# maoqingyu1996/Boosting-Neural-Video-Representation-via-Online-Structural-Reparameteration

Hardware: AMD Instinct MI355X
Metric: training frames/sec, Bunny 720p ERB (higher is better)
Workload: dtype f16; 1 GPU; configs[1]: Bunny-shaped 132x3x720x1280 synthetic video, branch_type=ERB, fc_hw_dim 9_16_26, strides 5 2 2 2 2, stem 512_1, lower_width 96, Fusion6, Adam(0.5,0.999), b=1; one independent video per GPU; precision=fp16, hip_graph=False, launch_mode=stream, finite=True

## Files before the change

boosting-neural-video-representation-via-online-structural-reparameteration_amd/_lib.py:

```python
import ctypes
import os
from ctypes import POINTER, c_char_p, c_double, c_float, c_int, c_int32, c_int64, c_size_t, c_void_p

HERE = os.path.dirname(os.path.abspath(__file__))
ORN_MAX_LAYERS = 8
LOSS_TYPES = {'L2': 0, 'L1': 1, 'Fusion6': 2}


class OrnError(RuntimeError):
    pass


def lib_path() -> str:
    return os.environ.get('ORN_LIB_PATH') or os.path.join(HERE, 'liborn.so')


class LayerDesc(ctypes.Structure):
    _fields_ = [('C', c_int32), ('O', c_int32), ('s', c_int32), ('H', c_int32), ('W', c_int32),
                ('w3x3', c_int64), ('b3x3', c_int64), ('w3x1', c_int64), ('b3x1', c_int64),
                ('w1x3', c_int64), ('b1x3', c_int64), ('w1', c_int64), ('w2', c_int64), ('w3', c_int64)]


class EngineDesc(ctypes.Structure):
    _fields_ = [('n_layers', c_int32), ('erb', c_int32), ('embed_len', c_int32), ('stem_dim', c_int32),
                ('fc_h', c_int32), ('fc_w', c_int32), ('fc_dim', c_int32), ('sigmoid', c_int32),
                ('loss_type', c_int32), ('precision', c_int32),
                ('beta1', c_double), ('beta2', c_double), ('eps', c_double),
                ('stem_w0', c_int64), ('stem_b0', c_int64), ('stem_w1', c_int64), ('stem_b1', c_int64),
                ('head_w', c_int64), ('head_b', c_int64), ('n_params', c_int64),
                ('layer', LayerDesc * ORN_MAX_LAYERS)]


P = c_void_p
_SIGS = {
    'orn_version': (c_int, []),
    'orn_last_error': (c_int, [c_char_p, c_size_t]),
    'orn_pe_fwd': (c_int, [P, c_int, P, c_int, P, P]),
    'orn_stem_fwd': (c_int, [P, P, P, P, P, c_int, c_int, c_int, c_int, P, P, P, P, P]),
    'orn_stem_bwd': (c_int, [P, P, P, P, P, P, c_int, c_int, c_int, c_int, P, P, P, P, P, P]),
    'orn_erb_merge_fwd': (c_int, [P] * 9 + [c_int, c_int, P, P, P, P]),
    'orn_erb_merge_bwd_ws_bytes': (c_size_t, [c_int, c_int]),
    'orn_erb_merge_bwd': (c_int, [P] * 6 + [c_int, c_int] + [P] * 9 + [P, c_size_t, P]),
    'orn_conv3x3_ps_silu_fwd': (c_int, [P, P, P, c_int, c_int, c_int, c_int, c_int, c_int, P, P, P]),
    'orn_conv3x3_ps_silu_bwd_ws_bytes': (c_size_t, [c_int] * 5),
    'orn_conv3x3_ps_silu_bwd': (c_int, [P, P, P, P] + [c_int] * 6 + [P, P, P, P, c_size_t, P]),
    'orn_conv3x3_ps_silu_bf16_ws_bytes': (c_size_t, [c_int] * 5),
    'orn_conv3x3_ps_silu_fwd_bf16': (c_int, [P, P, P] + [c_int] * 5 + [P, P, P, c_size_t, P]),
    'orn_conv3x3_ps_silu_bwd_bf16': (c_int, [P, P, P, P] + [c_int] * 5 + [P, P, P, P, c_size_t, P]),
    'orn_conv_nhwc_bf16_fwd': (c_int, [P, P, P] + [c_int] * 5 + [P, P, P]),
    'orn_conv_nhwc_f16_fwd': (c_int, [P, P, P] + [c_int] * 5 + [P, P, P]),
    'orn_dgrad_nhwc_bf16': (c_int, [P, P] + [c_int] * 4 + [P, P, c_int, P]),
    'orn_wgrad_nhwc_bf16_ws_bytes': (c_size_t, [c_int] * 3),
    'orn_wgrad_nhwc_bf16': (c_int, [P, P] + [c_int] * 5 + [P, P, P, P]),
    'orn_dgrad_nhwc_f16': (c_int, [P, P] + [c_int] * 4 + [P, P, c_int, P]),
    'orn_wgrad_nhwc_f16': (c_int, [P, P] + [c_int] * 5 + [P, P, P, P]),
    'orn_conv3x3_ps_silu_fwd_f16': (c_int, [P, P, P] + [c_int] * 5 + [P, P, P, c_size_t, P]),
    'orn_conv3x3_ps_silu_bwd_f16': (c_int, [P, P, P, P] + [c_int] * 5 + [P, P, P, P, c_size_t, P]),
    'orn_head_fwd': (c_int, [P, P, P, c_int, c_int, c_int, c_int, c_int, P, P]),
    'orn_head_bwd_ws_bytes': (c_size_t, [c_int] * 4),
    'orn_head_bwd': (c_int, [P, P, P, P, c_int, c_int, c_int, c_int, c_int, P, P, P, P, c_size_t, P]),
    'orn_loss_ws_bytes': (c_size_t, [c_int] * 4),
    'orn_loss_fwd_bwd': (c_int, [P, P, c_int, c_int, c_int, c_int, c_int, c_float, P, P, P, c_size_t, P]),
    'orn_loss_target_stats_bytes': (c_size_t, [c_int] * 4),
    'orn_loss_target_stats': (c_int, [P, c_int, c_int, c_int, c_int, P, P]),
    'orn_msssim_ws_bytes': (c_size_t, [c_int] * 4),
    'orn_msssim': (c_int, [P, P, c_int, c_int, c_int, c_int, P, P, c_size_t, P]),
    'orn_adam_step': (c_int, [P, P, P, P, c_size_t, c_double, c_double, c_double, c_double, c_int, P]),
    'orn_engine_ws_bytes': (c_size_t, [POINTER(EngineDesc)]),
    'orn_engine_create': (c_int, [POINTER(EngineDesc), P, P, P, P, P, c_size_t, POINTER(c_void_p)]),
    'orn_engine_destroy': (None, [P]),
    'orn_engine_decode': (c_int, [P, P, P, P]),
    'orn_engine_train_step': (c_int, [P, P, P, P, P, P, c_int32, P]),
    'orn_engine_train_steps_graph': (c_int, [P, P, P, P, P, P, c_int32, c_int32, P]),
    'orn_engine_train_steps': (c_int, [P, P, P, P, P, P, c_int32, c_int32, P]),
    'orn_engine_profile_step': (c_int, [P, P, P, P, P, P, c_int32, P, P]),
    'orn_engine_set_grad_mask': (c_int, [P, P]),
    'orn_engine_set_target_stats': (c_int, [P, P]),
    'orn_engine_fused_kernel': (c_int, [P, c_int, POINTER(c_void_p), POINTER(c_void_p)]),
    'orn_engine_scale_state': (c_int, [P, P]),
    'orn_engine_set_grad_scale': (c_int, [P, c_float, c_float]),
}
EXPORTS = tuple(_SIGS.keys())
_DEBUG_SIGS = {'orn_debug_set': (None, [c_int]), 'orn_debug_set_stamps': (None, [c_void_p]),
               'orn_debug_conv_fwd_bf16': (c_int, [P, P, P] + [c_int] * 5 + [P, P, c_int, P]),
               'orn_debug_conv_fwd_f16': (c_int, [P, P, P] + [c_int] * 5 + [P, P, c_int, P]),
               'orn_debug_conv_dgrad_bf16': (c_int, [P, P] + [c_int] * 4 + [P, P, c_int, P, c_int, P]),
               'orn_debug_conv_dgrad_f16': (c_int, [P, P] + [c_int] * 4 + [P, P, c_int, P, c_int, P]),
               'orn_debug_merge_h16_bwd': (c_int, [c_int, P, P, P, P, P])}

_lib = None


def lib():
    global _lib
    if _lib is None:
        path = lib_path()
        if not os.path.exists(path):
            raise OrnError(f'{path} is missing: build it with `python -c "import __graft_entry__ as g; g.build()"` '
                           '(hipcc --offload-arch=gfx950).  There is no CPU fallback.')
        L = ctypes.CDLL(path)
        for name, (res, args) in _SIGS.items():
            fn = getattr(L, name)
            fn.restype = res
            fn.argtypes = args
        for name, (res, args) in _DEBUG_SIGS.items():
            fn = getattr(L, name, None)
            if fn is not None:
                fn.restype = res
                fn.argtypes = args
        _lib = L
    return _lib


def last_error() -> str:
    buf = ctypes.create_string_buffer(512)
    lib().orn_last_error(buf, 512)
    return buf.value.decode('utf-8', 'replace')


def check(rc: int, what: str = ''):
    if rc != 0:
        raise OrnError(f'{what or "liborn"} failed (rc={rc}): {last_error()}')


def ptr(t):
    if t is None:
        return None
    if not t.is_cuda:
        raise OrnError('liborn ops need tensors on the GPU (there is no CPU path)')
    if not t.is_contiguous():
        raise OrnError('liborn ops need contiguous tensors')
    return c_void_p(t.data_ptr())


def stream():
    import torch
    return c_void_p(torch.cuda.current_stream().cuda_stream)
```

boosting-neural-video-representation-via-online-structural-reparameteration_amd/csrc/orn_loss.hip:

```cpp
#include "orn_internal.h"

#define SS_TH 16
#define SS_TW 64
#define SS_PH (SS_TH + 10)
#define SS_PW (SS_TW + 10)
#define SS_PWP 76

__constant__ float c_gauss[11];

struct LossP {
    const float *pred, *target;
    const int *frame_idx;
    size_t frame_stride;
    int planes, H, W, Hv, Wv;
    float *part_ssim;
    float *part_l1;
    float *dpred;
    int loss_type;
    int vec4;
    float *tstats;
    size_t tstats_stride;
    float g_l1, g_l2, g_ssim;
    int tiles_w, tiles_h;
};

#define F6_TH 16
#define F6_TW 64
#define F6_PH (F6_TH + 20)
#define F6_PWP 88
#define F6_DH (F6_TH + 10)
#define F6_DWP 76
#define F6_LDS_FLOATS (2 * F6_PH * F6_PWP + 5 * F6_PH * F6_DWP + 16)

enum { TC_NONE = 0, TC_READ = 1, TC_FILL = 2 };
template <bool GRAD, int TC>
__global__ void __launch_bounds__(256) k_fusion6(LossP q)
{
    extern __shared__ __attribute__((aligned(16))) float f6s[];
    float *Xp = f6s, *Xt = f6s + F6_PH * F6_PWP;
    float *Hm = f6s + 2 * F6_PH * F6_PWP;
    float *Dm = f6s;
    float *Hh = Hm;
    float *sred = f6s + 2 * F6_PH * F6_PWP + 5 * F6_PH * F6_DWP;
    const int t = threadIdx.x;
    const int plane = blockIdx.y;
    const int tw = blockIdx.x % q.tiles_w, th = blockIdx.x / q.tiles_w;
    const int y0 = th * F6_TH, x0 = tw * F6_TW;
    const size_t HW = (size_t)q.H * q.W;
    const size_t fr = TC == TC_FILL ? (size_t)blockIdx.z : (q.frame_idx ? (size_t)(*q.frame_idx) : 0);
    const float *tp = q.target + fr * q.frame_stride + (size_t)plane * HW;
    const float *pp = TC == TC_FILL ? tp : q.pred + (size_t)plane * HW;
    float *ts_mu = nullptr, *ts_tt = nullptr;
    if (TC != TC_NONE) {
        ts_mu = q.tstats + fr * q.tstats_stride + (size_t)plane * q.Hv * q.Wv;
        ts_tt = ts_mu + (size_t)q.planes * q.Hv * q.Wv;
    }
    constexpr int RPT = 9;
    const int vrg = t / F6_DWP, vj = t - vrg * F6_DWP, vr4 = vrg == 2 ? 17 : vrg * RPT;
    float c_mu[RPT], c_tt[RPT];
    if (TC == TC_READ && t < 3 * F6_DWP) {
#pragma unroll
        for (int o = 0; o < RPT; ++o) {
            const int vy = min(max(y0 - 10 + vr4 + o, 0), q.Hv - 1), vx = min(max(x0 - 10 + vj, 0), q.Wv - 1);
            c_mu[o] = ts_mu[(size_t)vy * q.Wv + vx];
            c_tt[o] = ts_tt[(size_t)vy * q.Wv + vx];
        }
    }
    if (q.vec4) {
        constexpr int NU = 22, NIT = (F6_PH * NU + 255) / 256;
        float4 ra[NIT], rb[NIT];
#pragma unroll
        for (int it = 0; it < NIT; ++it) {
            const int idx = t + it * 256;
            const int r = idx / NU, u = idx - r * NU;
            const int gy = y0 - 10 + r, gx = x0 - 12 + 4 * u;
            ra[it] = make_float4(0.f, 0.f, 0.f, 0.f); rb[it] = ra[it];
            if (idx < F6_PH * NU && gy >= 0 && gy < q.H && gx >= 0 && gx < q.W) {
                ra[it] = *reinterpret_cast<const float4 *>(pp + (size_t)gy * q.W + gx);
                rb[it] = *reinterpret_cast<const float4 *>(tp + (size_t)gy * q.W + gx);
            }
        }
#pragma unroll
        for (int it = 0; it < NIT; ++it) {
            const int idx = t + it * 256;
            const int r = idx / NU, u = idx - r * NU;
            if (idx < F6_PH * NU) {
                const int c = 4 * u - 2;
                if (u > 0) {
                    *reinterpret_cast<float2 *>(Xp + r * F6_PWP + c) = make_float2(ra[it].x, ra[it].y);
                    *reinterpret_cast<float2 *>(Xt + r * F6_PWP + c) = make_float2(rb[it].x, rb[it].y);
                }
                *reinterpret_cast<float2 *>(Xp + r * F6_PWP + c + 2) = make_float2(ra[it].z, ra[it].w);
                *reinterpret_cast<float2 *>(Xt + r * F6_PWP + c + 2) = make_float2(rb[it].z, rb[it].w);
            }
        }
    } else {
        constexpr int NL = (F6_PH * F6_PWP + 255) / 256;
#pragma unroll 1
        for (int it = 0; it < NL; ++it) {
            const int idx = t + it * 256;
            const int r = idx / F6_PWP, c = idx - r * F6_PWP;
            const int gy = y0 - 10 + r, gx = x0 - 10 + c;
            float a = 0.f, b = 0.f;
            if (idx < F6_PH * F6_PWP && gy >= 0 && gy < q.H && gx >= 0 && gx < q.W) { a = pp[(size_t)gy * q.W + gx]; b = tp[(size_t)gy * q.W + gx]; }
            if (idx < F6_PH * F6_PWP) { Xp[idx] = a; Xt[idx] = b; }
        }
    }
    __syncthreads();
    for (int idx = t; idx < F6_PH * (F6_DWP / 4); idx += 256) {
        const int r = idx / (F6_DWP / 4), c4 = (idx - r * (F6_DWP / 4)) * 4;
        float a[16], b[16];
#pragma unroll
        for (int k = 0; k < 4; ++k) {
            const float4 va = *reinterpret_cast<const float4 *>(Xp + r * F6_PWP + c4 + 4 * k);
            const float4 vb = *reinterpret_cast<const float4 *>(Xt + r * F6_PWP + c4 + 4 * k);
            a[4 * k] = va.x; a[4 * k + 1] = va.y; a[4 * k + 2] = va.z; a[4 * k + 3] = va.w;
            b[4 * k] = vb.x; b[4 * k + 1] = vb.y; b[4 * k + 2] = vb.z; b[4 * k + 3] = vb.w;
        }
        float sp[4] = {0, 0, 0, 0}, st[4] = {0, 0, 0, 0}, spp[4] = {0, 0, 0, 0}, stt[4] = {0, 0, 0, 0}, spt[4] = {0, 0, 0, 0};
        constexpr bool P_MAPS = TC != TC_FILL, T_MAPS = TC != TC_READ;
#pragma unroll
        for (int k = 0; k < 14; ++k) {
            const float aa = a[k] * a[k], bb = b[k] * b[k], ab = a[k] * b[k];
#pragma unroll
            for (int o = 0; o < 4; ++o) {
                const int tap = k - o;
                if (tap >= 0 && tap < 11) {
                    const float g = c_gauss[tap];
                    if (P_MAPS) { sp[o] = fmaf(g, a[k], sp[o]); spp[o] = fmaf(g, aa, spp[o]); spt[o] = fmaf(g, ab, spt[o]); }
                    if (T_MAPS) { st[o] = fmaf(g, b[k], st[o]); stt[o] = fmaf(g, bb, stt[o]); }
                }
            }
        }
        float *h = Hm + r * F6_DWP + c4;
        if (P_MAPS) {
            *reinterpret_cast<float4 *>(h) = make_float4(sp[0], sp[1], sp[2], sp[3]);
            *reinterpret_cast<float4 *>(h + 2 * F6_PH * F6_DWP) = make_float4(spp[0], spp[1], spp[2], spp[3]);
            *reinterpret_cast<float4 *>(h + 4 * F6_PH * F6_DWP) = make_float4(spt[0], spt[1], spt[2], spt[3]);
        }
        if (T_MAPS) {
            *reinterpret_cast<float4 *>(h + F6_PH * F6_DWP) = make_float4(st[0], st[1], st[2], st[3]);
            *reinterpret_cast<float4 *>(h + 3 * F6_PH * F6_DWP) = make_float4(stt[0], stt[1], stt[2], stt[3]);
        }
    }
    __syncthreads();
    const float C1 = 0.01f * 0.01f, C2 = 0.03f * 0.03f;
    float ssum = 0.f;
    if (t < 3 * F6_DWP) {
        const int rg = vrg, j = vj, r4 = vr4;
        float v[5][RPT];
#pragma unroll
        for (int m = 0; m < 5; ++m) {
            if ((TC == TC_READ && (m == 1 || m == 3)) || (TC == TC_FILL && !(m == 1 || m == 3))) continue;
            float col[RPT + 10];
#pragma unroll
            for (int k = 0; k < RPT + 10; ++k) col[k] = Hm[(m * F6_PH + r4 + k) * F6_DWP + j];
#pragma unroll
            for (int o = 0; o < RPT; ++o) {
                float acc = 0.f;
#pragma unroll
                for (int k = 0; k < 11; ++k) acc = fmaf(c_gauss[k], col[o + k], acc);
                v[m][o] = acc;
            }
        }
#pragma unroll
        for (int o = 0; o < RPT; ++o) {
            const int i = r4 + o;
            const int vy = y0 - 10 + i, vx = x0 - 10 + j;
            float dm = 0.f, dq = 0.f, dr = 0.f;
            if (TC == TC_FILL) {
                if (vy >= 0 && vy < q.Hv && vx >= 0 && vx < q.Wv && i >= 10 && j >= 10 && j < F6_TW + 10 && (rg < 2 || o > 0)) {
                    ts_mu[(size_t)vy * q.Wv + vx] = v[1][o];
                    ts_tt[(size_t)vy * q.Wv + vx] = v[3][o];
                }
                continue;
            }
            if (vy >= 0 && vy < q.Hv && vx >= 0 && vx < q.Wv && j < F6_TW + 10) {
                const float m = v[0][o], qq = v[2][o], rr = v[4][o];
                const float mu = TC == TC_READ ? c_mu[o] : v[1][o];
                const float tt = TC == TC_READ ? c_tt[o] : v[3][o];
                const float sp = qq - m * m, st = tt - mu * mu, spt = rr - m * mu;
                const float A1 = 2.f * m * mu + C1, A2 = 2.f * spt + C2;
                const float B1 = m * m + mu * mu + C1, B2 = sp + st + C2;
                float i1 = __builtin_amdgcn_rcpf(B1), i2 = __builtin_amdgcn_rcpf(B2);
                i1 = i1 * (2.0f - B1 * i1);
                i2 = i2 * (2.0f - B2 * i2);
                const float inv = i1 * i2;
                const float S = A1 * A2 * inv;
                if (i >= 10 && j >= 10 && (rg < 2 || o > 0)) ssum += S;
                dm = 2.f * mu * (A2 - A1) * inv - 2.f * m * S * i1 + 2.f * m * S * i2;
                dq = -S * i2;
                dr = 2.f * A1 * inv;
            }
            float *d = Dm + i * F6_DWP + j;
            d[0] = dm; d[F6_DH * F6_DWP] = dq; d[2 * F6_DH * F6_DWP] = dr;
        }
    }
    if (TC == TC_FILL) return;
    const int fc = t & (F6_TW - 1), fr4 = (t >> 6) * 4;
    float fp[4], ft[4];
#pragma unroll
    for (int o = 0; o < 4; ++o) {
        const size_t oo = (size_t)min(y0 + fr4 + o, q.H - 1) * q.W + min(x0 + fc, q.W - 1);
        fp[o] = pp[oo]; ft[o] = tp[oo];
    }
    __syncthreads();
    float sabs = 0.f, ssq = 0.f;
    if (GRAD) {
        for (int idx = t; idx < F6_DH * (F6_TW / 4); idx += 256) {
            const int r = idx / (F6_TW / 4), c4 = (idx - r * (F6_TW / 4)) * 4;
#pragma unroll
            for (int m = 0; m < 3; ++m) {
                float w[16];
#pragma unroll
                for (int k = 0; k < 4; ++k) {
                    const float4 vv = *reinterpret_cast<const float4 *>(Dm + (m * F6_DH + r) * F6_DWP + c4 + 4 * k);
                    w[4 * k] = vv.x; w[4 * k + 1] = vv.y; w[4 * k + 2] = vv.z; w[4 * k + 3] = vv.w;
                }
                float hv[4];
#pragma unroll
                for (int o = 0; o < 4; ++o) {
                    float acc = 0.f;
#pragma unroll
                    for (int k = 0; k < 11; ++k) acc = fmaf(c_gauss[k], w[o + 10 - k], acc);
                    hv[o] = acc;
                }
                *reinterpret_cast<float4 *>(Hh + (m * F6_DH + r) * F6_TW + c4) = make_float4(hv[0], hv[1], hv[2], hv[3]);
            }
        }
        __syncthreads();
    }
    {
        const int c = fc, r4 = fr4;
        float am[4] = {0, 0, 0, 0}, aq[4] = {0, 0, 0, 0}, ar[4] = {0, 0, 0, 0};
        if (GRAD) {
#pragma unroll
            for (int m = 0; m < 3; ++m) {
                float col[14];
#pragma unroll
                for (int k = 0; k < 14; ++k) col[k] = Hh[(m * F6_DH + r4 + k) * F6_TW + c];
#pragma unroll
                for (int o = 0; o < 4; ++o) {
                    float acc = 0.f;
#pragma unroll
                    for (int k = 0; k < 11; ++k) acc = fmaf(c_gauss[k], col[o + 10 - k], acc);
                    if (m == 0) am[o] = acc; else if (m == 1) aq[o] = acc; else ar[o] = acc;
                }
            }
        }
        const int gx = x0 + c;
#pragma unroll
        for (int o = 0; o < 4; ++o) {
            const int gy = y0 + r4 + o;
            if (gy >= q.H || gx >= q.W) continue;
            const size_t oo = (size_t)gy * q.W + gx;
            const float p = fp[o], tg = ft[o], d = p - tg;
            sabs += fabsf(d);
            ssq = fmaf(d, d, ssq);
            if (GRAD) {
                float g = q.g_l1 * ((d > 0.f) ? 1.f : ((d < 0.f) ? -1.f : 0.f));
                g -= q.g_ssim * (am[o] + 2.f * p * aq[o] + tg * ar[o]);
                q.dpred[(size_t)plane * HW + oo] = g;
            }
        }
    }
    const float ts = orn_block_sum(ssum, sred);
    const float ta = orn_block_sum(sabs, sred);
    const float tq = orn_block_sum(ssq, sred);
    if (t == 0) {
        const size_t bi = (size_t)plane * gridDim.x + blockIdx.x;
        q.part_ssim[bi] = ts;
        q.part_l1[2 * bi] = ta;
        q.part_l1[2 * bi + 1] = tq;
    }
}

template <int LT, bool GRAD>
__global__ void __launch_bounds__(256) k_loss_grad(LossP q)
{
    __shared__ float sred[16];
    const int t = threadIdx.x;
    const int plane = blockIdx.y;
    const int tw = blockIdx.x % q.tiles_w, th = blockIdx.x / q.tiles_w;
    const int y0 = th * SS_TH, x0 = tw * SS_TW;
    const size_t HW = (size_t)q.H * q.W;
    const float *pp = q.pred + (size_t)plane * HW;
    const float *tp = q.target + (q.frame_idx ? (size_t)(*q.frame_idx) * q.frame_stride : 0) + (size_t)plane * HW;
    float sabs = 0.f, ssq = 0.f;
    for (int idx = t; idx < SS_TH * SS_TW; idx += 256) {
        const int r = idx / SS_TW, c = idx - r * SS_TW;
        const int gy = y0 + r, gx = x0 + c;
        if (gy >= q.H || gx >= q.W) continue;
        const size_t o = (size_t)gy * q.W + gx;
        const float p = pp[o], tg = tp[o], d = p - tg;
        sabs += fabsf(d);
        ssq = fmaf(d, d, ssq);
        if (GRAD) {
            float g;
            if (LT == ORN_LOSS_L2) g = q.g_l2 * d;
            else g = q.g_l1 * ((d > 0.f) ? 1.f : ((d < 0.f) ? -1.f : 0.f));
            q.dpred[(size_t)plane * HW + o] = g;
        }
    }
    const float ta = orn_block_sum(sabs, sred);
    const float tq = orn_block_sum(ssq, sred);
    if (t == 0) {
        const size_t bi = (size_t)plane * gridDim.x + blockIdx.x;
        q.part_l1[2 * bi] = ta;
        q.part_l1[2 * bi + 1] = tq;
    }
}

__global__ void __launch_bounds__(256) k_loss_finalize(OrnLossFinalJob j)
{
    __shared__ double sd[3 * 256];
    orn_loss_finalize_block(j, sd);
}

static bool g_gauss_ready = false;

static int ensure_gauss()
{
    if (g_gauss_ready) return 0;
    float g[11], s = 0.f;
    for (int i = 0; i < 11; ++i) {
        const float c = (float)(i - 5);
        g[i] = expf(-(c * c) / (2.0f * 1.5f * 1.5f));
        s += g[i];
    }
    for (int i = 0; i < 11; ++i) g[i] /= s;
    hipError_t e = hipMemcpyToSymbol(HIP_SYMBOL(c_gauss), g, sizeof(g));
    if (e != hipSuccess) {
        orn_set_error("loss: hipMemcpyToSymbol failed: %s", hipGetErrorString(e));
        return (int)e;
    }
    g_gauss_ready = true;
    return 0;
}

struct LossGeom { int planes, Hv, Wv, tw, th; size_t nmap, off_pl, total; };

static LossGeom loss_geom(int B, int Ch, int H, int W)
{
    LossGeom g;
    g.planes = B * Ch;
    g.Hv = H > 10 ? H - 10 : 0;
    g.Wv = W > 10 ? W - 10 : 0;
    g.tw = orn_cdiv(W, SS_TW); g.th = orn_cdiv(H, SS_TH);
    g.nmap = (size_t)g.planes * g.Hv * g.Wv;
    g.off_pl = orn_align((size_t)g.planes * g.tw * g.th * 4 + 4) / 4;
    g.total = g.off_pl + orn_align((size_t)g.planes * g.tw * g.th * 8 + 8) / 4;
    return g;
}

extern "C" size_t orn_loss_ws_bytes(int B, int Ch, int H, int W) { return loss_geom(B, Ch, H, W).total * 4; }

static int ensure_fusion6_lds()
{
    static bool done = false;
    if (done) return 0;
    hipError_t e = hipSuccess;
    const void *kerns[] = {(const void *)k_fusion6<true, TC_NONE>, (const void *)k_fusion6<false, TC_NONE>, (const void *)k_fusion6<true, TC_READ>,
                           (const void *)k_fusion6<false, TC_READ>, (const void *)k_fusion6<false, TC_FILL>};
    for (const void *k : kerns)
        if (e == hipSuccess) e = hipFuncSetAttribute(k, hipFuncAttributeMaxDynamicSharedMemorySize, F6_LDS_FLOATS * 4);
    if (e != hipSuccess) { orn_set_error("loss: hipFuncSetAttribute: %s", hipGetErrorString(e)); return (int)e; }
    done = true;
    return 0;
}

int orn_loss_init() { ORN_TRY(ensure_gauss()); return ensure_fusion6_lds(); }

int orn_launch_loss(const float *pred, const float *target, const int *frame_idx, size_t frame_stride, int B, int Ch,
                    int H, int W, int loss_type, float loss_scale, float *stats, float *dpred, float *ws,
                    hipStream_t st, const OrnStepCur *cur, float *ring, OrnScaleState *sc, const float *tstats, OrnLossFinalJob *defer)
{
    ORN_REQUIRE(loss_type == ORN_LOSS_L2 || loss_type == ORN_LOSS_L1 || loss_type == ORN_LOSS_FUSION6,
                "loss: unsupported loss_type %d", loss_type);
    ORN_TRY(orn_loss_init());
    static_assert(SS_TH == F6_TH && SS_TW == F6_TW, "one tiling for all loss kernels");
    const LossGeom g = loss_geom(B, Ch, H, W);
    if (loss_type == ORN_LOSS_FUSION6) ORN_REQUIRE(g.Hv > 0 && g.Wv > 0, "loss: SSIM needs H,W > 10 (got %dx%d)", H, W);
    LossP q;
    q.pred = pred; q.target = target; q.frame_idx = frame_idx; q.frame_stride = frame_stride;
    q.planes = g.planes; q.H = H; q.W = W; q.Hv = g.Hv; q.Wv = g.Wv;
    q.part_ssim = ws; q.part_l1 = ws + g.off_pl;
    q.dpred = dpred; q.loss_type = loss_type;
    q.tstats = const_cast<float *>(tstats); q.tstats_stride = 2 * g.nmap;
    q.vec4 = (W % 4 == 0 && ((uintptr_t)pred | (uintptr_t)target) % 16 == 0 && (frame_stride % 4 == 0 || !frame_idx)) ? 1 : 0;
    const double n = (double)g.planes * H * W;
    q.g_l1 = (float)((loss_type == ORN_LOSS_FUSION6 ? 0.7 : 1.0) * loss_scale / n);
    q.g_l2 = (float)(2.0 * loss_scale / n);
    q.g_ssim = g.nmap ? (float)(0.3 * loss_scale / (double)g.nmap) : 0.f;
    q.tiles_w = g.tw; q.tiles_h = g.th;
    const int n_tiles = g.planes * g.tw * g.th;
    {
        const dim3 gr(g.tw * g.th, g.planes), bl(256);
        const bool gd = q.dpred != nullptr;
        if (loss_type == ORN_LOSS_FUSION6) {
            if (tstats) { if (gd) hipLaunchKernelGGL((k_fusion6<true, TC_READ>), gr, bl, F6_LDS_FLOATS * 4, st, q); else hipLaunchKernelGGL((k_fusion6<false, TC_READ>), gr, bl, F6_LDS_FLOATS * 4, st, q); }
            else if (gd) hipLaunchKernelGGL((k_fusion6<true, TC_NONE>), gr, bl, F6_LDS_FLOATS * 4, st, q); else hipLaunchKernelGGL((k_fusion6<false, TC_NONE>), gr, bl, F6_LDS_FLOATS * 4, st, q);
        }
        else if (loss_type == ORN_LOSS_L2) { if (gd) hipLaunchKernelGGL((k_loss_grad<ORN_LOSS_L2, true>), gr, bl, 0, st, q); else hipLaunchKernelGGL((k_loss_grad<ORN_LOSS_L2, false>), gr, bl, 0, st, q); }
        else { if (gd) hipLaunchKernelGGL((k_loss_grad<ORN_LOSS_L1, true>), gr, bl, 0, st, q); else hipLaunchKernelGGL((k_loss_grad<ORN_LOSS_L1, false>), gr, bl, 0, st, q); }
    }
    ORN_LAUNCH_CHECK("loss");
    const OrnLossFinalJob fj = {q.part_ssim, loss_type == ORN_LOSS_FUSION6 ? n_tiles : 0, q.part_l1, n_tiles, n, (double)g.nmap, loss_type,
                                loss_scale, stats, cur, ring, sc};
    if (defer) { *defer = fj; return 0; }
    hipLaunchKernelGGL(k_loss_finalize, dim3(1), dim3(256), 0, st, fj);
    ORN_LAUNCH_CHECK("loss_finalize");
    return 0;
}

extern "C" size_t orn_loss_target_stats_bytes(int n, int Ch, int H, int W)
{
    if (n <= 0 || Ch <= 0 || H <= 10 || W <= 10) return 0;
    return (size_t)n * 2 * Ch * (H - 10) * (W - 10) * sizeof(float);
}

extern "C" int orn_loss_target_stats(const float *frames, int n, int Ch, int H, int W, float *out, void *stream)
{
    ORN_REQUIRE(frames && out && n > 0 && Ch > 0 && H > 10 && W > 10 && n <= 65535, "loss_target_stats: bad arguments");
    ORN_TRY(orn_loss_init());
    const LossGeom g = loss_geom(1, Ch, H, W);
    LossP q = {};
    q.pred = frames; q.target = frames; q.frame_idx = nullptr; q.frame_stride = (size_t)Ch * H * W;
    q.planes = g.planes; q.H = H; q.W = W; q.Hv = g.Hv; q.Wv = g.Wv;
    q.tstats = out; q.tstats_stride = 2 * g.nmap;
    q.loss_type = ORN_LOSS_FUSION6;
    q.vec4 = (W % 4 == 0 && (uintptr_t)frames % 16 == 0) ? 1 : 0;
    q.tiles_w = g.tw; q.tiles_h = g.th;
    hipLaunchKernelGGL((k_fusion6<false, TC_FILL>), dim3(g.tw * g.th, g.planes, n), dim3(256), F6_LDS_FLOATS * 4, (hipStream_t)stream, q);
    ORN_LAUNCH_CHECK("loss_target_stats");
    return 0;
}

extern "C" int orn_loss_fwd_bwd(const float *pred, const float *target, int B, int Ch, int H, int W, int loss_type,
                                float loss_scale, float *stats, float *dpred, void *ws, size_t ws_bytes,
                                void *stream)
{
    ORN_REQUIRE(pred && target && stats && ws, "loss_fwd_bwd: null pointer");
    ORN_REQUIRE(B > 0 && Ch > 0 && H > 0 && W > 0, "loss_fwd_bwd: bad sizes");
    if (ws_bytes < orn_loss_ws_bytes(B, Ch, H, W)) {
        orn_set_error("loss_fwd_bwd: workspace %zu < %zu", ws_bytes, orn_loss_ws_bytes(B, Ch, H, W));
        return ORN_E_WS;
    }
    return orn_launch_loss(pred, target, nullptr, 0, B, Ch, H, W, loss_type, loss_scale, stats, dpred, (float *)ws,
                           (hipStream_t)stream, nullptr, nullptr);
}

__global__ void __launch_bounds__(256)
k_ssim_cs_partial(const float *__restrict__ x, const float *__restrict__ y, int H, int W, int tiles_w, float *__restrict__ part)
{
    __shared__ __attribute__((aligned(16))) float Ps[SS_PH][SS_PWP];
    __shared__ __attribute__((aligned(16))) float Ts[SS_PH][SS_PWP];
    __shared__ float Hs[5][SS_PH][SS_TW];
    __shared__ float sred[16];
    const int t = threadIdx.x, plane = blockIdx.y;
    const int tw = blockIdx.x % tiles_w, th = blockIdx.x / tiles_w;
    const int y0 = th * SS_TH, x0 = tw * SS_TW;
    const int Hv = H - 10, Wv = W - 10;
    const float *pp = x + (size_t)plane * H * W, *tp = y + (size_t)plane * H * W;
    for (int idx = t; idx < SS_PH * SS_PWP; idx += 256) {
        const int r = idx / SS_PWP, c = idx - r * SS_PWP;
        const int gy = y0 + r, gx = x0 + c;
        const bool ok = c < SS_PW && gy < H && gx < W;
        Ps[r][c] = ok ? pp[(size_t)gy * W + gx] : 0.f;
        Ts[r][c] = ok ? tp[(size_t)gy * W + gx] : 0.f;
    }
    __syncthreads();
    for (int idx = t; idx < SS_PH * SS_TW; idx += 256) {
        const int r = idx / SS_TW, c = idx - r * SS_TW;
        float sp = 0.f, st = 0.f, spp = 0.f, stt = 0.f, spt = 0.f;
#pragma unroll
        for (int k = 0; k < 11; ++k) {
            const float g = c_gauss[k], a = Ps[r][c + k], b = Ts[r][c + k];
            sp = fmaf(g, a, sp); st = fmaf(g, b, st);
            spp = fmaf(g, a * a, spp); stt = fmaf(g, b * b, stt); spt = fmaf(g, a * b, spt);
        }
        Hs[0][r][c] = sp; Hs[1][r][c] = st; Hs[2][r][c] = spp; Hs[3][r][c] = stt; Hs[4][r][c] = spt;
    }
    __syncthreads();
    const float C1 = 0.01f * 0.01f, C2 = 0.03f * 0.03f;
    float ss = 0.f, cs = 0.f;
    for (int idx = t; idx < SS_TH * SS_TW; idx += 256) {
        const int r = idx / SS_TW, c = idx - r * SS_TW;
        if (y0 + r >= Hv || x0 + c >= Wv) continue;
        float m = 0.f, mu = 0.f, qq = 0.f, tt = 0.f, rr = 0.f;
#pragma unroll
        for (int k = 0; k < 11; ++k) {
            const float g = c_gauss[k];
            m = fmaf(g, Hs[0][r + k][c], m); mu = fmaf(g, Hs[1][r + k][c], mu);
            qq = fmaf(g, Hs[2][r + k][c], qq); tt = fmaf(g, Hs[3][r + k][c], tt); rr = fmaf(g, Hs[4][r + k][c], rr);
        }
        const float csm = (2.f * (rr - m * mu) + C2) / ((qq - m * m) + (tt - mu * mu) + C2);
        cs += csm;
        ss += ((2.f * m * mu + C1) / (m * m + mu * mu + C1)) * csm;
    }
    const float a = orn_block_sum(ss, sred);
    const float b = orn_block_sum(cs, sred);
    if (t == 0) {
        const size_t bi = (size_t)plane * gridDim.x + blockIdx.x;
        part[2 * bi] = a;
        part[2 * bi + 1] = b;
    }
}

__global__ void k_avgpool2(const float *__restrict__ in, int planes, int H, int W, int Ho, int Wo, int ph, int pw, float *__restrict__ out)
{
    const size_t idx = (size_t)blockIdx.x * blockDim.x + threadIdx.x;
    if (idx >= (size_t)planes * Ho * Wo) return;
    const int xo = (int)(idx % Wo), yo = (int)((idx / Wo) % Ho), pl = (int)(idx / ((size_t)Wo * Ho));
    const float *p = in + (size_t)pl * H * W;
    float s = 0.f;
#pragma unroll
    for (int dy = 0; dy < 2; ++dy)
#pragma unroll
        for (int dx = 0; dx < 2; ++dx) {
            const int yy = yo * 2 + dy - ph, xx = xo * 2 + dx - pw;
            if (yy >= 0 && yy < H && xx >= 0 && xx < W) s += p[(size_t)yy * W + xx];
        }
    out[idx] = s * 0.25f;
}

__global__ void k_msssim_finalize(const float *__restrict__ part, const int *__restrict__ nblk, const float *__restrict__ nmap,
                                  int planes, float *__restrict__ out)
{
    __shared__ double acc[64];
    const float wts[5] = {0.0448f, 0.2856f, 0.3001f, 0.2363f, 0.1333f};
    const int pl = threadIdx.x;
    double val = 0.0;
    if (pl < planes) {
        size_t off = 0;
        double prod = 1.0;
        for (int lv = 0; lv < 5; ++lv) {
            double ss = 0.0, cs = 0.0;
            for (int b = 0; b < nblk[lv]; ++b) {
                ss += (double)part[off + 2 * ((size_t)pl * nblk[lv] + b)];
                cs += (double)part[off + 2 * ((size_t)pl * nblk[lv] + b) + 1];
            }
            off += (size_t)2 * planes * nblk[lv];
            const double v = (lv < 4 ? cs : ss) / (double)nmap[lv];
            prod *= pow(v > 0.0 ? v : 0.0, (double)wts[lv]);
        }
        val = prod;
    }
    acc[pl] = val;
    __syncthreads();
    if (pl == 0) {
        double s = 0.0;
        for (int i = 0; i < planes; ++i) s += acc[i];
        out[0] = (float)(s / planes);
    }
}

static void msssim_geom(int H, int W, int Hs[5], int Ws[5])
{
    Hs[0] = H; Ws[0] = W;
    for (int l = 1; l < 5; ++l) { Hs[l] = (Hs[l - 1] + 2 * (Hs[l - 1] % 2)) / 2; Ws[l] = (Ws[l - 1] + 2 * (Ws[l - 1] % 2)) / 2; }
}

extern "C" size_t orn_msssim_ws_bytes(int B, int Ch, int H, int W)
{
    int Hs[5], Ws[5];
    msssim_geom(H, W, Hs, Ws);
    const size_t planes = (size_t)B * Ch;
    size_t f = 64;
    for (int l = 1; l < 5; ++l) f += 2 * orn_align(planes * Hs[l] * Ws[l] * 4) / 4;
    for (int l = 0; l < 5; ++l) f += orn_align(2 * planes * orn_cdiv(Ws[l] - 10, SS_TW) * orn_cdiv(Hs[l] - 10, SS_TH) * 4 + 8) / 4;
    return f * 4;
}

extern "C" int orn_msssim(const float *pred, const float *target, int B, int Ch, int H, int W, float *out, void *ws,
                          size_t ws_bytes, void *stream)
{
    ORN_REQUIRE(pred && target && out && ws, "msssim: null pointer");
    ORN_REQUIRE(B > 0 && Ch > 0 && B * Ch <= 64, "msssim: bad plane count");
    ORN_REQUIRE((H < W ? H : W) > 160, "msssim: image side must exceed 160 (got %dx%d)", H, W);
    if (ws_bytes < orn_msssim_ws_bytes(B, Ch, H, W)) { orn_set_error("msssim: workspace too small"); return ORN_E_WS; }
    ORN_TRY(ensure_gauss());
    hipStream_t st = (hipStream_t)stream;
    int Hs[5], Ws[5];
    msssim_geom(H, W, Hs, Ws);
    const int planes = B * Ch;
    float *base = (float *)ws;
    int *d_nblk = (int *)base;
    float *d_nmap = base + 8;
    float *cur = base + 64;
    const float *x = pred, *y = target;
    int h_nblk[5];
    float h_nmap[5];
    float *pooled[5][2] = {};
    for (int l = 1; l < 5; ++l)
        for (int k = 0; k < 2; ++k) { pooled[l][k] = cur; cur += orn_align((size_t)planes * Hs[l] * Ws[l] * 4) / 4; }
    float *part = cur;
    size_t poff = 0;
    for (int l = 0; l < 5; ++l) {
        const int tw = orn_cdiv(Ws[l] - 10, SS_TW), th = orn_cdiv(Hs[l] - 10, SS_TH);
        h_nblk[l] = tw * th;
        h_nmap[l] = (float)(Hs[l] - 10) * (float)(Ws[l] - 10);
        hipLaunchKernelGGL(k_ssim_cs_partial, dim3(tw * th, planes), dim3(256), 0, st, x, y, Hs[l], Ws[l], tw, part + poff);
        ORN_LAUNCH_CHECK("ssim_cs_partial");
        poff += (size_t)2 * planes * h_nblk[l];
        if (l < 4) {
            const size_t n = (size_t)planes * Hs[l + 1] * Ws[l + 1];
            hipLaunchKernelGGL(k_avgpool2, dim3(orn_cdiv((long)n, 256)), dim3(256), 0, st, x, planes, Hs[l], Ws[l], Hs[l + 1], Ws[l + 1],
                               Hs[l] % 2, Ws[l] % 2, pooled[l + 1][0]);
            hipLaunchKernelGGL(k_avgpool2, dim3(orn_cdiv((long)n, 256)), dim3(256), 0, st, y, planes, Hs[l], Ws[l], Hs[l + 1], Ws[l + 1],
                               Hs[l] % 2, Ws[l] % 2, pooled[l + 1][1]);
            ORN_LAUNCH_CHECK("avgpool2");
            x = pooled[l + 1][0];
            y = pooled[l + 1][1];
        }
    }
    hipError_t rc = hipMemcpyAsync(d_nblk, h_nblk, sizeof(h_nblk), hipMemcpyHostToDevice, st);
    if (rc == hipSuccess) rc = hipMemcpyAsync(d_nmap, h_nmap, sizeof(h_nmap), hipMemcpyHostToDevice, st);
    if (rc == hipSuccess) rc = hipStreamSynchronize(st);
    if (rc != hipSuccess) { orn_set_error("msssim: table upload failed: %s", hipGetErrorString(rc)); return (int)rc; }
    hipLaunchKernelGGL(k_msssim_finalize, dim3(1), dim3(64), 0, st, part, d_nblk, d_nmap, planes, out);
    ORN_LAUNCH_CHECK("msssim_finalize");
    return 0;
}
```

include/orn_debug.h:

```cpp
#ifndef ORN_DEBUG_H_
#define ORN_DEBUG_H_
#include "orn.h"
#ifdef __cplusplus
extern "C" {
#endif
ORN_API void orn_debug_set(int flags);
ORN_API int orn_debug_conv_fwd_bf16(const void *xpad, const void *wb, const float *bias_p, int H, int W, int Cin, int O, int s,
                                    void *z, void *apad, int c_real, void *stream);
ORN_API int orn_debug_conv_fwd_f16(const void *xpad, const void *wb, const float *bias_p, int H, int W, int Cin, int O, int s,
                                   void *z, void *apad, int c_real, void *stream);
ORN_API int orn_debug_conv_dgrad_bf16(const void *dypad, const void *wd, int H, int W, int O, int C, const void *zprev,
                                      void *dyprev, int sp, float *dx_f32, int c_real, void *stream);
ORN_API int orn_debug_conv_dgrad_f16(const void *dypad, const void *wd, int H, int W, int O, int C, const void *zprev,
                                     void *dyprev, int sp, float *dx_f32, int c_real, void *stream);
ORN_API int orn_debug_merge_h16_bwd(int n, const int *co, const float *const *in, float *const *out, int *flag, void *stream);
#ifdef ORN_CONV_STAMP
ORN_API void orn_debug_set_stamps(void *buf);
#endif
#ifdef __cplusplus
}
#endif
#endif
```

Measured before the change: 948.8 frames/s.

## Enlarge Fusion6 loss tile height and trim LDS to fit two groups per CU

Raises the Fusion6 SSIM/L1 loss tile from 16 to 30 rows, so the 10-row halo is amortised over more output rows and fewer redundant blur computations and loads are done. The LDS layout is resized per variant: the cached-target-stats form keeps only three horizontal maps and overlaps the halo buffers, so two work-groups still fit per CU. Per-thread row counts and ownership masks are generalised to the new geometry. It also adds a debug entry point for the cached variant. Larger tiles mean fewer blocks and more registers per thread, which risks lower occupancy or load imbalance on the 720-row frame.

```diff
diff --git a/boosting-neural-video-representation-via-online-structural-reparameteration_amd/_lib.py b/boosting-neural-video-representation-via-online-structural-reparameteration_amd/_lib.py
--- a/boosting-neural-video-representation-via-online-structural-reparameteration_amd/_lib.py
+++ b/boosting-neural-video-representation-via-online-structural-reparameteration_amd/_lib.py
@@ -86,7 +86,8 @@
                'orn_debug_conv_fwd_f16': (c_int, [P, P, P] + [c_int] * 5 + [P, P, c_int, P]),
                'orn_debug_conv_dgrad_bf16': (c_int, [P, P] + [c_int] * 4 + [P, P, c_int, P, c_int, P]),
                'orn_debug_conv_dgrad_f16': (c_int, [P, P] + [c_int] * 4 + [P, P, c_int, P, c_int, P]),
-               'orn_debug_merge_h16_bwd': (c_int, [c_int, P, P, P, P, P])}
+               'orn_debug_merge_h16_bwd': (c_int, [c_int, P, P, P, P, P]),
+               'orn_debug_loss_fusion6_cached': (c_int, [P, P, P] + [c_int] * 4 + [c_float, P, P, P, c_size_t, P])}
 
 _lib = None
 
diff --git a/boosting-neural-video-representation-via-online-structural-reparameteration_amd/csrc/orn_loss.hip b/boosting-neural-video-representation-via-online-structural-reparameteration_amd/csrc/orn_loss.hip
--- a/boosting-neural-video-representation-via-online-structural-reparameteration_amd/csrc/orn_loss.hip
+++ b/boosting-neural-video-representation-via-online-structural-reparameteration_amd/csrc/orn_loss.hip
@@ -1,10 +1,4 @@
 #include "orn_internal.h"
-
-#define SS_TH 16
-#define SS_TW 64
-#define SS_PH (SS_TH + 10)
-#define SS_PW (SS_TW + 10)
-#define SS_PWP 76
 
 __constant__ float c_gauss[11];
 
@@ -24,28 +18,43 @@
     int tiles_w, tiles_h;
 };
 
-#define F6_TH 16
-#define F6_TW 64
-#define F6_PH (F6_TH + 20)
-#define F6_PWP 88
-#define F6_DH (F6_TH + 10)
-#define F6_DWP 76
-#define F6_LDS_FLOATS (2 * F6_PH * F6_PWP + 5 * F6_PH * F6_DWP + 16)
+#ifndef ORN_F6_TH
+#define ORN_F6_TH 30
+#endif
+constexpr int LS_TH = ORN_F6_TH, LS_TW = 64;
+constexpr int F6_PH = LS_TH + 20, F6_PWP = 88;
+constexpr int F6_DH = LS_TH + 10, F6_DW = LS_TW + 10, F6_DWP = 76;
+constexpr int F6_XF = 2 * F6_PH * F6_PWP > 3 * F6_DH * F6_DWP ? 2 * F6_PH * F6_PWP : 3 * F6_DH * F6_DWP;
+constexpr int F6_NRG = 256 / F6_DW;
+constexpr int F6_RPT = (F6_DH + F6_NRG - 1) / F6_NRG;
+constexpr int F6_FR = (LS_TH + 3) / 4;
+constexpr int F6_LDS_CU = 160 * 1024;
 
 enum { TC_NONE = 0, TC_READ = 1, TC_FILL = 2 };
+constexpr int f6_maps(int tc) { return tc == TC_READ ? 3 : (tc == TC_FILL ? 2 : 5); }
+constexpr int f6_slot(int tc, int m) { return tc == TC_READ ? m / 2 : (tc == TC_FILL ? (m - 1) / 2 : m); }
+constexpr int f6_lds_floats(int tc, int hwp) { return F6_XF + f6_maps(tc) * F6_PH * hwp + 16; }
+constexpr int f6_hwp(int tc) { return f6_lds_floats(tc, 76) * 4 <= F6_LDS_CU / 2 ? 76 : 74; }
+constexpr int f6_lds_bytes(int tc) { return f6_lds_floats(tc, f6_hwp(tc)) * 4; }
+static_assert(LS_TH >= 4 && LS_TW == 64 && F6_XF % 4 == 0 && F6_NRG >= 1, "k_fusion6: tile geometry");
+static_assert(3 * F6_DH * LS_TW <= 3 * F6_PH * 74, "k_fusion6: Hh must fit over the three maps of TC_READ");
+static_assert(f6_lds_bytes(TC_READ) <= F6_LDS_CU / 2, "k_fusion6: the timed form must run two work-groups per CU");
+static_assert(f6_lds_bytes(TC_NONE) <= F6_LDS_CU && f6_lds_bytes(TC_FILL) <= F6_LDS_CU, "k_fusion6: LDS of a CU");
+
 template <bool GRAD, int TC>
 __global__ void __launch_bounds__(256) k_fusion6(LossP q)
 {
+    constexpr int HWP = f6_hwp(TC), HMAP = F6_PH * HWP;
     extern __shared__ __attribute__((aligned(16))) float f6s[];
     float *Xp = f6s, *Xt = f6s + F6_PH * F6_PWP;
-    float *Hm = f6s + 2 * F6_PH * F6_PWP;
+    float *Hm = f6s + F6_XF;
     float *Dm = f6s;
     float *Hh = Hm;
-    float *sred = f6s + 2 * F6_PH * F6_PWP + 5 * F6_PH * F6_DWP;
+    float *sred = Hm + f6_maps(TC) * HMAP;
     const int t = threadIdx.x;
     const int plane = blockIdx.y;
     const int tw = blockIdx.x % q.tiles_w, th = blockIdx.x / q.tiles_w;
-    const int y0 = th * F6_TH, x0 = tw * F6_TW;
+    const int y0 = th * LS_TH, x0 = tw * LS_TW;
     const size_t HW = (size_t)q.H * q.W;
     const size_t fr = TC == TC_FILL ? (size_t)blockIdx.z : (q.frame_idx ? (size_t)(*q.frame_idx) : 0);
     const float *tp = q.target + fr * q.frame_stride + (size_t)plane * HW;
@@ -55,10 +64,10 @@
         ts_mu = q.tstats + fr * q.tstats_stride + (size_t)plane * q.Hv * q.Wv;
         ts_tt = ts_mu + (size_t)q.planes * q.Hv * q.Wv;
     }
-    constexpr int RPT = 9;
-    const int vrg = t / F6_DWP, vj = t - vrg * F6_DWP, vr4 = vrg == 2 ? 17 : vrg * RPT;
+    constexpr int RPT = F6_RPT;
+    const int vrg = t / F6_DW, vj = t - vrg * F6_DW, vr4 = min(vrg * RPT, F6_DH - RPT);
     float c_mu[RPT], c_tt[RPT];
-    if (TC == TC_READ && t < 3 * F6_DWP) {
+    if (TC == TC_READ && t < F6_NRG * F6_DW) {
 #pragma unroll
         for (int o = 0; o < RPT; ++o) {
             const int vy = min(max(y0 - 10 + vr4 + o, 0), q.Hv - 1), vx = min(max(x0 - 10 + vj, 0), q.Wv - 1);
@@ -132,21 +141,22 @@
                 }
             }
         }
-        float *h = Hm + r * F6_DWP + c4;
-        if (P_MAPS) {
-            *reinterpret_cast<float4 *>(h) = make_float4(sp[0], sp[1], sp[2], sp[3]);
-            *reinterpret_cast<float4 *>(h + 2 * F6_PH * F6_DWP) = make_float4(spp[0], spp[1], spp[2], spp[3]);
-            *reinterpret_cast<float4 *>(h + 4 * F6_PH * F6_DWP) = make_float4(spt[0], spt[1], spt[2], spt[3]);
-        }
-        if (T_MAPS) {
-            *reinterpret_cast<float4 *>(h + F6_PH * F6_DWP) = make_float4(st[0], st[1], st[2], st[3]);
-            *reinterpret_cast<float4 *>(h + 3 * F6_PH * F6_DWP) = make_float4(stt[0], stt[1], stt[2], stt[3]);
-        }
+        float *h = Hm + r * HWP + c4;
+        auto put = [&](int m, const float *v) {
+            float *d = h + f6_slot(TC, m) * HMAP;
+            if (HWP % 4 == 0) *reinterpret_cast<float4 *>(d) = make_float4(v[0], v[1], v[2], v[3]);
+            else {
+                *reinterpret_cast<float2 *>(d) = make_float2(v[0], v[1]);
+                if (c4 + 2 < HWP) *reinterpret_cast<float2 *>(d + 2) = make_float2(v[2], v[3]);
+            }
+        };
+        if (P_MAPS) { put(0, sp); put(2, spp); put(4, spt); }
+        if (T_MAPS) { put(1, st); put(3, stt); }
     }
     __syncthreads();
     const float C1 = 0.01f * 0.01f, C2 = 0.03f * 0.03f;
     float ssum = 0.f;
-    if (t < 3 * F6_DWP) {
+    if (t < F6_NRG * F6_DW) {
         const int rg = vrg, j = vj, r4 = vr4;
         float v[5][RPT];
 #pragma unroll
@@ -154,7 +164,7 @@
             if ((TC == TC_READ && (m == 1 || m == 3)) || (TC == TC_FILL && !(m == 1 || m == 3))) continue;
             float col[RPT + 10];
 #pragma unroll
-            for (int k = 0; k < RPT + 10; ++k) col[k] = Hm[(m * F6_PH + r4 + k) * F6_DWP + j];
+            for (int k = 0; k < RPT + 10; ++k) col[k] = Hm[f6_slot(TC, m) * HMAP + (r4 + k) * HWP + j];
 #pragma unroll
             for (int o = 0; o < RPT; ++o) {
                 float acc = 0.f;
@@ -166,16 +176,17 @@
 #pragma unroll
         for (int o = 0; o < RPT; ++o) {
             const int i = r4 + o;
+            const bool own = i >= 10 && i >= rg * RPT && j >= 10;
             const int vy = y0 - 10 + i, vx = x0 - 10 + j;
             float dm = 0.f, dq = 0.f, dr = 0.f;
             if (TC == TC_FILL) {
-                if (vy >= 0 && vy < q.Hv && vx >= 0 && vx < q.Wv && i >= 10 && j >= 10 && j < F6_TW + 10 && (rg < 2 || o > 0)) {
+                if (vy >= 0 && vy < q.Hv && vx >= 0 && vx < q.Wv && own) {
                     ts_mu[(size_t)vy * q.Wv + vx] = v[1][o];
                     ts_tt[(size_t)vy * q.Wv + vx] = v[3][o];
                 }
                 continue;
             }
-            if (vy >= 0 && vy < q.Hv && vx >= 0 && vx < q.Wv && j < F6_TW + 10) {
+            if (vy >= 0 && vy < q.Hv && vx >= 0 && vx < q.Wv) {
                 const float m = v[0][o], qq = v[2][o], rr = v[4][o];
                 const float mu = TC == TC_READ ? c_mu[o] : v[1][o];
                 const float tt = TC == TC_READ ? c_tt[o] : v[3][o];
@@ -187,7 +198,7 @@
                 i2 = i2 * (2.0f - B2 * i2);
                 const float inv = i1 * i2;
                 const float S = A1 * A2 * inv;
-                if (i >= 10 && j >= 10 && (rg < 2 || o > 0)) ssum += S;
+                if (own) ssum += S;
                 dm = 2.f * mu * (A2 - A1) * inv - 2.f * m * S * i1 + 2.f * m * S * i2;
                 dq = -S * i2;
                 dr = 2.f * A1 * inv;
@@ -197,18 +208,19 @@
         }
     }
     if (TC == TC_FILL) return;
-    const int fc = t & (F6_TW - 1), fr4 = (t >> 6) * 4;
-    float fp[4], ft[4];
-#pragma unroll
-    for (int o = 0; o < 4; ++o) {
+    constexpr int FR = F6_FR;
+    const int fc = t & (LS_TW - 1), fr4 = (t >> 6) * FR;
+    float fp[FR], ft[FR];
+#pragma unroll
+    for (int o = 0; o < FR; ++o) {
         const size_t oo = (size_t)min(y0 + fr4 + o, q.H - 1) * q.W + min(x0 + fc, q.W - 1);
         fp[o] = pp[oo]; ft[o] = tp[oo];
     }
     __syncthreads();
     float sabs = 0.f, ssq = 0.f;
     if (GRAD) {
-        for (int idx = t; idx < F6_DH * (F6_TW / 4); idx += 256) {
-            const int r = idx / (F6_TW / 4), c4 = (idx - r * (F6_TW / 4)) * 4;
+        for (int idx = t; idx < F6_DH * (LS_TW / 4); idx += 256) {
+            const int r = idx / (LS_TW / 4), c4 = (idx - r * (LS_TW / 4)) * 4;
 #pragma unroll
             for (int m = 0; m < 3; ++m) {
                 float w[16];
@@ -225,22 +237,22 @@
                     for (int k = 0; k < 11; ++k) acc = fmaf(c_gauss[k], w[o + 10 - k], acc);
                     hv[o] = acc;
                 }
-                *reinterpret_cast<float4 *>(Hh + (m * F6_DH + r) * F6_TW + c4) = make_float4(hv[0], hv[1], hv[2], hv[3]);
+                *reinterpret_cast<float4 *>(Hh + (m * F6_DH + r) * LS_TW + c4) = make_float4(hv[0], hv[1], hv[2], hv[3]);
             }
         }
         __syncthreads();
     }
     {
         const int c = fc, r4 = fr4;
-        float am[4] = {0, 0, 0, 0}, aq[4] = {0, 0, 0, 0}, ar[4] = {0, 0, 0, 0};
+        float am[FR] = {}, aq[FR] = {}, ar[FR] = {};
         if (GRAD) {
 #pragma unroll
             for (int m = 0; m < 3; ++m) {
-                float col[14];
-#pragma unroll
-                for (int k = 0; k < 14; ++k) col[k] = Hh[(m * F6_DH + r4 + k) * F6_TW + c];
-#pragma unroll
-                for (int o = 0; o < 4; ++o) {
+                float col[FR + 10];
+#pragma unroll
+                for (int k = 0; k < FR + 10; ++k) col[k] = Hh[(m * F6_DH + min(r4 + k, F6_DH - 1)) * LS_TW + c];
+#pragma unroll
+                for (int o = 0; o < FR; ++o) {
                     float acc = 0.f;
 #pragma unroll
                     for (int k = 0; k < 11; ++k) acc = fmaf(c_gauss[k], col[o + 10 - k], acc);
@@ -250,9 +262,9 @@
         }
         const int gx = x0 + c;
 #pragma unroll
-        for (int o = 0; o < 4; ++o) {
+        for (int o = 0; o < FR; ++o) {
             const int gy = y0 + r4 + o;
-            if (gy >= q.H || gx >= q.W) continue;
+            if (r4 + o >= LS_TH || gy >= q.H || gx >= q.W) continue;
             const size_t oo = (size_t)gy * q.W + gx;
             const float p = fp[o], tg = ft[o], d = p - tg;
             sabs += fabsf(d);
@@ -282,13 +294,13 @@
     const int t = threadIdx.x;
     const int plane = blockIdx.y;
     const int tw = blockIdx.x % q.tiles_w, th = blockIdx.x / q.tiles_w;
-    const int y0 = th * SS_TH, x0 = tw * SS_TW;
+    const int y0 = th * LS_TH, x0 = tw * LS_TW;
     const size_t HW = (size_t)q.H * q.W;
     const float *pp = q.pred + (size_t)plane * HW;
     const float *tp = q.target + (q.frame_idx ? (size_t)(*q.frame_idx) * q.frame_stride : 0) + (size_t)plane * HW;
     float sabs = 0.f, ssq = 0.f;
-    for (int idx = t; idx < SS_TH * SS_TW; idx += 256) {
-        const int r = idx / SS_TW, c = idx - r * SS_TW;
+    for (int idx = t; idx < LS_TH * LS_TW; idx += 256) {
+        const int r = idx / LS_TW, c = idx - r * LS_TW;
         const int gy = y0 + r, gx = x0 + c;
         if (gy >= q.H || gx >= q.W) continue;
         const size_t o = (size_t)gy * q.W + gx;
@@ -346,7 +358,7 @@
     g.planes = B * Ch;
     g.Hv = H > 10 ? H - 10 : 0;
     g.Wv = W > 10 ? W - 10 : 0;
-    g.tw = orn_cdiv(W, SS_TW); g.th = orn_cdiv(H, SS_TH);
+    g.tw = orn_cdiv(W, LS_TW); g.th = orn_cdiv(H, LS_TH);
     g.nmap = (size_t)g.planes * g.Hv * g.Wv;
     g.off_pl = orn_align((size_t)g.planes * g.tw * g.th * 4 + 4) / 4;
     g.total = g.off_pl + orn_align((size_t)g.planes * g.tw * g.th * 8 + 8) / 4;
@@ -360,10 +372,12 @@
     static bool done = false;
     if (done) return 0;
     hipError_t e = hipSuccess;
-    const void *kerns[] = {(const void *)k_fusion6<true, TC_NONE>, (const void *)k_fusion6<false, TC_NONE>, (const void *)k_fusion6<true, TC_READ>,
-                           (const void *)k_fusion6<false, TC_READ>, (const void *)k_fusion6<false, TC_FILL>};
-    for (const void *k : kerns)
-        if (e == hipSuccess) e = hipFuncSetAttribute(k, hipFuncAttributeMaxDynamicSharedMemorySize, F6_LDS_FLOATS * 4);
+    const struct { const void *k; int bytes; } kerns[] = {
+        {(const void *)k_fusion6<true, TC_NONE>, f6_lds_bytes(TC_NONE)}, {(const void *)k_fusion6<false, TC_NONE>, f6_lds_bytes(TC_NONE)},
+        {(const void *)k_fusion6<true, TC_READ>, f6_lds_bytes(TC_READ)}, {(const void *)k_fusion6<false, TC_READ>, f6_lds_bytes(TC_READ)},
+        {(const void *)k_fusion6<false, TC_FILL>, f6_lds_bytes(TC_FILL)}};
+    for (const auto &kn : kerns)
+        if (e == hipSuccess) e = hipFuncSetAttribute(kn.k, hipFuncAttributeMaxDynamicSharedMemorySize, kn.bytes);
     if (e != hipSuccess) { orn_set_error("loss: hipFuncSetAttribute: %s", hipGetErrorString(e)); return (int)e; }
     done = true;
     return 0;
@@ -378,7 +392,6 @@
     ORN_REQUIRE(loss_type == ORN_LOSS_L2 || loss_type == ORN_LOSS_L1 || loss_type == ORN_LOSS_FUSION6,
                 "loss: unsupported loss_type %d", loss_type);
     ORN_TRY(orn_loss_init());
-    static_assert(SS_TH == F6_TH && SS_TW == F6_TW, "one tiling for all loss kernels");
     const LossGeom g = loss_geom(B, Ch, H, W);
     if (loss_type == ORN_LOSS_FUSION6) ORN_REQUIRE(g.Hv > 0 && g.Wv > 0, "loss: SSIM needs H,W > 10 (got %dx%d)", H, W);
     LossP q;
@@ -398,8 +411,8 @@
         const dim3 gr(g.tw * g.th, g.planes), bl(256);
         const bool gd = q.dpred != nullptr;
         if (loss_type == ORN_LOSS_FUSION6) {
-            if (tstats) { if (gd) hipLaunchKernelGGL((k_fusion6<true, TC_READ>), gr, bl, F6_LDS_FLOATS * 4, st, q); else hipLaunchKernelGGL((k_fusion6<false, TC_READ>), gr, bl, F6_LDS_FLOATS * 4, st, q); }
-            else if (gd) hipLaunchKernelGGL((k_fusion6<true, TC_NONE>), gr, bl, F6_LDS_FLOATS * 4, st, q); else hipLaunchKernelGGL((k_fusion6<false, TC_NONE>), gr, bl, F6_LDS_FLOATS * 4, st, q);
+            if (tstats) { if (gd) hipLaunchKernelGGL((k_fusion6<true, TC_READ>), gr, bl, f6_lds_bytes(TC_READ), st, q); else hipLaunchKernelGGL((k_fusion6<false, TC_READ>), gr, bl, f6_lds_bytes(TC_READ), st, q); }
+            else if (gd) hipLaunchKernelGGL((k_fusion6<true, TC_NONE>), gr, bl, f6_lds_bytes(TC_NONE), st, q); else hipLaunchKernelGGL((k_fusion6<false, TC_NONE>), gr, bl, f6_lds_bytes(TC_NONE), st, q);
         }
         else if (loss_type == ORN_LOSS_L2) { if (gd) hipLaunchKernelGGL((k_loss_grad<ORN_LOSS_L2, true>), gr, bl, 0, st, q); else hipLaunchKernelGGL((k_loss_grad<ORN_LOSS_L2, false>), gr, bl, 0, st, q); }
         else { if (gd) hipLaunchKernelGGL((k_loss_grad<ORN_LOSS_L1, true>), gr, bl, 0, st, q); else hipLaunchKernelGGL((k_loss_grad<ORN_LOSS_L1, false>), gr, bl, 0, st, q); }
@@ -431,7 +444,7 @@
     q.loss_type = ORN_LOSS_FUSION6;
     q.vec4 = (W % 4 == 0 && (uintptr_t)frames % 16 == 0) ? 1 : 0;
     q.tiles_w = g.tw; q.tiles_h = g.th;
-    hipLaunchKernelGGL((k_fusion6<false, TC_FILL>), dim3(g.tw * g.th, g.planes, n), dim3(256), F6_LDS_FLOATS * 4, (hipStream_t)stream, q);
+    hipLaunchKernelGGL((k_fusion6<false, TC_FILL>), dim3(g.tw * g.th, g.planes, n), dim3(256), f6_lds_bytes(TC_FILL), (hipStream_t)stream, q);
     ORN_LAUNCH_CHECK("loss_target_stats");
     return 0;
 }
@@ -450,6 +463,24 @@
                            (hipStream_t)stream, nullptr, nullptr);
 }
 
+extern "C" int orn_debug_loss_fusion6_cached(const float *pred, const float *target, const float *tstats, int B, int Ch, int H, int W,
+                                             float loss_scale, float *stats, float *dpred, void *ws, size_t ws_bytes, void *stream)
+{
+    ORN_REQUIRE(pred && target && tstats && stats && ws, "loss_fusion6_cached: null pointer");
+    ORN_REQUIRE(B > 0 && Ch > 0 && H > 10 && W > 10, "loss_fusion6_cached: bad sizes");
+    if (ws_bytes < orn_loss_ws_bytes(B, Ch, H, W)) {
+        orn_set_error("loss_fusion6_cached: workspace %zu < %zu", ws_bytes, orn_loss_ws_bytes(B, Ch, H, W));
+        return ORN_E_WS;
+    }
+    return orn_launch_loss(pred, target, nullptr, 0, B, Ch, H, W, ORN_LOSS_FUSION6, loss_scale, stats, dpred, (float *)ws,
+                           (hipStream_t)stream, nullptr, nullptr, nullptr, tstats);
+}
+
+#define SS_TH 16
+#define SS_TW 64
+#define SS_PH (SS_TH + 10)
+#define SS_PW (SS_TW + 10)
+#define SS_PWP 76
 __global__ void __launch_bounds__(256)
 k_ssim_cs_partial(const float *__restrict__ x, const float *__restrict__ y, int H, int W, int tiles_w, float *__restrict__ part)
 {
diff --git a/include/orn_debug.h b/include/orn_debug.h
--- a/include/orn_debug.h
+++ b/include/orn_debug.h
@@ -14,6 +14,8 @@
 ORN_API int orn_debug_conv_dgrad_f16(const void *dypad, const void *wd, int H, int W, int O, int C, const void *zprev,
                                      void *dyprev, int sp, float *dx_f32, int c_real, void *stream);
 ORN_API int orn_debug_merge_h16_bwd(int n, const int *co, const float *const *in, float *const *out, int *flag, void *stream);
+ORN_API int orn_debug_loss_fusion6_cached(const float *pred, const float *target, const float *tstats, int B, int Ch, int H, int W,
+                                          float loss_scale, float *stats, float *dpred, void *ws, size_t ws_bytes, void *stream);
 #ifdef ORN_CONV_STAMP
 ORN_API void orn_debug_set_stamps(void *buf);
 #endif
```

Result: no change. 958.3 frames/s, median of 6 (+1.0%).
